# ChumpChief/FluidFramework

Measured on AMD Instinct MI355X. Metric: sequenced ops applied/sec (whole node) + achieved HBM GB/s, conflict-farm replay, higher is better.
Workload: dtype int32

## Files before the change

fluidframework_amd/csrc/mt_engine.h:

```cpp
#pragma once

#include "../../include/fmt.h"
#include "wave.h"
#include "adjust.h"
#include "huge_ckpt.h"

#include <cstddef>
#include <type_traits>

#if FMT_GPU
#define FMT_LDS __attribute__((address_space(3)))
#else
#define FMT_LDS
#endif

namespace fmt_mt {

constexpr int kMaxNodes = 8;
constexpr int kGranularity = 256;
constexpr int kObCap = 64;
constexpr int kKeysMax = FMT_MT_PROPS_KEYS_MAX;
constexpr int kKeyChunks = kKeysMax / 64;
static_assert(kKeysMax % 64 == 0, "prop-set slots come in whole waves");
constexpr int32_t kNotRemoved = 0x7fffffff;
constexpr int kCapacityFinal = -33;
constexpr int kCkptEscalate = -34;
constexpr int kCkptDescend = -36;
constexpr int kDescendLeaves4 = 128, kDescendChars4 = 1024;
constexpr int kDescendMinOps = 128;

struct SmallTier {
  static constexpr int kRows = 8;
  static constexpr int kCapChars = 6144;
  static constexpr int kMaxBlocks = 128;
  static constexpr int kHeapCap = 255;
  static constexpr int kPropCap = 32;
  static constexpr int kLenBits = 16, kBlkBits = 8;
  static constexpr bool kHbmChars = false;
  static constexpr bool kUnroll = true;
  static constexpr int kWords = 5;
  static constexpr int kMaxClient = 31;
  static constexpr bool kPropsWord = false;
  using BId = uint8_t;
  using VR = V8;
};

struct CompactTier : SmallTier {
  static constexpr int kRows = 4;
  static constexpr int kCapChars = 2048;
  using VR = V4;
};

struct MicroTier : SmallTier {
  static constexpr int kRows = 2;
  static constexpr int kCapChars = 1024;
  using VR = V2;
};

struct LargeTier {
  static constexpr int kRows = 32;
  static constexpr int kCapChars = 131071;
  static constexpr int kMaxBlocks = 1023;
  static constexpr int kHeapCap = 1023;
  static constexpr int kPropCap = 1024;
  static constexpr int kLenBits = 17, kBlkBits = 10;
  static constexpr bool kHbmChars = true;
  static constexpr bool kUnroll = false;
  static constexpr int kWords = 7;
  static constexpr int kMaxClient = 63;
  static constexpr bool kPropsWord = true;
  using BId = uint16_t;
  using VR = V32;
};

#define FMT_PRAGMA(x) _Pragma(#x)
#define FOR_ROWS(r, lo, hi)                                                                            \
  FMT_PRAGMA(unroll kRowUnroll)                                                                      \
  for (int r = kRowUnroll > 1 ? 0 : (lo); r < (kRowUnroll > 1 ? kRows : ((hi) < kRows ? (hi) : kRows)); r++) \
    if (r >= (lo) && r < (hi))
#define FOR_ROWS_DOWN(r, lo, hi)                                                                          \
  FMT_PRAGMA(unroll kRowUnroll)                                                                        \
  for (int r = kRowUnroll > 1 ? kRows - 1 : ((hi) < kRows ? (hi) : kRows) - 1; r >= (kRowUnroll > 1 ? 0 : (lo)); r--) \
    if (r >= (lo) && r < (hi))

template <class BId>
struct Blk {
  uint8_t count;
  BId parent;
  uint8_t leaf;
  int8_t needsScour;
  BId child[kMaxNodes];
};

struct HeapEnt {
  int32_t maxSeq;
  uint32_t leafId;
};

struct PropSet {
  uint32_t n;
  uint32_t kv[FMT_MT_PROPS_MAX];
};

struct ObEnt {
  uint32_t startId, endId;
  int32_t startOff, endOff;
  int32_t seq, client;
};

template <class C>
struct Scratch {
  uint16_t chars[C::kHbmChars ? 2 : C::kCapChars];
  Blk<typename C::BId> blk[C::kMaxBlocks];
  HeapEnt heap[C::kHeapCap + 1];
  PropSet props[C::kPropCap];
  uint16_t propCls[C::kPropCap];
  uint32_t kvWork[FMT_MT_PROPS_KEYS_MAX];
  typename C::BId freeList[C::kMaxBlocks];
  uint32_t tmp[64];
  ObEnt ob[kObCap];
  uint8_t obSeq[kObCap];
  uint8_t obStart[kObCap];
};

constexpr uint32_t kW4Marker = 1u << 23;
constexpr uint32_t kIdLimit = 1u << 23;
FMT_DEV uint32_t fId(uint32_t w4) { return w4 & 0x7FFFFFu; }
FMT_DEV bool fMarker(uint32_t w4) { return (w4 & kW4Marker) != 0; }
FMT_DEV int32_t fClient(uint32_t w4) { return static_cast<int32_t>(static_cast<int8_t>(w4 >> 24)); }
FMT_DEV uint32_t mkW4(uint32_t id, int32_t client) { return (id & 0x7FFFFFu) | (static_cast<uint32_t>(client & 0xFF) << 24); }

struct LeafRec {
  uint32_t w[8];
};

struct AdjustTables;

struct LocalTables {
  uint32_t* groups;
  const uint64_t* groupOffs;
  uint32_t* recs;
  const uint64_t* recOffs;
  uint32_t* pm;
  const uint64_t* pmOffs;
  fmt_mt_op* regen;
  const uint64_t* regenOffs;
  uint16_t* regenText;
  const uint64_t* regenTextOffs;
  uint32_t* regenCount;
  uint32_t* scratch;
  const uint64_t* scratchOffs;
};

struct DocInputs {
  const fmt_mt_op* ops;
  uint64_t begin, end;
  const uint16_t* text;
  uint32_t initOff, initLen;
  const uint32_t* propsOff;
  const uint32_t* propsKv;
  uint32_t nPropsOps;
  const fmt_mt_snapshot_seg* snapSegs;
  uint32_t nHeader, nBody;
  int32_t snapMinSeq, snapSeq;
  uint32_t loaded;
  const fmt_mt_snapshot_info* snapInfo;
  const fmt_mt_stamp* snapStamps;
  const fmt_mt_snapshot_info* infoAll;
  const fmt_mt_stamp* stampsAll;
  uint64_t nInfoAll;
  const fmt_mt_relpos* relpos;
  uint32_t nRelpos;
  uint32_t markerKey;
  const AdjustTables* adj;
  uint32_t doc;
  const LocalTables* loc = nullptr;
};

struct DocOutputs {
  fmt_mt_doc_result* header;
  fmt_mt_leaf* leaves;
  uint16_t* chars;
  fmt_mt_propset* props;
  fmt_mt_catchup_range* catchup;
  uint32_t catchupCap;
  fmt_mt_remove_order* rmOrder;
  uint32_t rmOrderCap;
  uint32_t* ckpt;
  bool ckptResume;
  uint32_t* bigCkpt;
  uint16_t* bigCkptChars;
  uint16_t* legacyProps;
  uint32_t* hugeCkpt = nullptr;
  bool descend = false;
};

#ifndef FMT_PROFILE
#define FMT_PROFILE 0
#endif
#ifndef FMT_SCALAR_OPS
#define FMT_SCALAR_OPS 0
#endif
enum ProfCat {
  kPfOpLoad, kPfScan, kPfSplit, kPfInsert, kPfRange, kPfLru, kPfZamboniOp, kPfWindow, kPfOutput,
  kPfInsChars, kPfInsShift, kPfZFind, kPfZChars, kPfZSerial, kPfZDelete, kPfZPack, kPfCount
};

template <bool Ob, class C = SmallTier, bool Rm = false, bool Adj = false, bool Loc = false>
class Doc {
 public:
  using VR = typename C::VR;
  using BId = typename C::BId;
  static constexpr int kRows = C::kRows;
  static constexpr int kRowUnroll = C::kUnroll ? C::kRows : 1;
  static constexpr int kCapLeaves = 64 * kRows;
  static constexpr int kCapChars = C::kCapChars;
  static constexpr int kMaxBlocks = C::kMaxBlocks;
  static constexpr int kHeapCap = C::kHeapCap;
  static constexpr int kPropCap = C::kPropCap;
  static constexpr uint32_t kLenMask = (1u << C::kLenBits) - 1u;
  static constexpr uint32_t kNoBlk = (1u << C::kBlkBits) - 1u;
  static constexpr bool kPW = C::kPropsWord;
  static constexpr int kCapFinal = C::kHbmChars ? FMT_E_CAPACITY : kCapacityFinal;
  static constexpr uint32_t kPropsUndef = kPW ? 0xFFFFu : (1u << (32 - C::kLenBits - C::kBlkBits)) - 1u;
  static_assert(kMaxBlocks <= static_cast<int>(kNoBlk) && kPropCap <= static_cast<int>(kPropsUndef), "W0 field widths");
  static_assert(kRows <= 32, "row bitmasks are 32-bit");
  FMT_DEV static uint32_t fLen(uint32_t w0) { return w0 & kLenMask; }
  FMT_DEV static uint32_t fBlk(uint32_t w0) { return (w0 >> C::kLenBits) & kNoBlk; }
  FMT_DEV static uint32_t fProps(uint32_t w0) { return kPW ? 0u : w0 >> (C::kLenBits + C::kBlkBits); }
  FMT_DEV static uint32_t mkW0(uint32_t len, uint32_t blk, uint32_t props) {
    return kPW ? len | (blk << C::kLenBits) : len | (blk << C::kLenBits) | (props << (C::kLenBits + C::kBlkBits));
  }

#if FMT_PROFILE && FMT_GPU
  uint64_t profT = 0;
  uint64_t prof[kPfCount] = {};
  FMT_DEV void stamp(int cat) {
    const uint64_t t = __builtin_amdgcn_s_memtime();
    prof[cat] += t - profT;
    profT = t;
  }
#else
  FMT_DEV void stamp(int) {}
#endif
  static constexpr int kWords = C::kWords + (Loc ? 1 : 0);
  static constexpr int kPropW = C::kWords - 1;
  static constexpr int kPendW = C::kWords;
  static constexpr int kMaxClient = C::kMaxClient;
  static constexpr int kTopClient = 253;
  Lane<VR> W[kWords];
  FMT_LDS Scratch<C>* s;
  uint16_t* gch = nullptr;
  int n = 0;
  int nChars = 0;
  int root = 0;
  int nFree = 0;
  int heapN = 0;
  int nProps = 0;
  int curSeq = 0;
  int minSeq = 0;
  int status = FMT_OK;
  int failSeq = 0;
  uint32_t nextId = 1;
  uint32_t opIdx = 0;
  int obSeqN = 0;
  int obStartN = 0;
  uint64_t obUsed = 0;
  uint32_t cuN = 0;
  DocInputs in;
  fmt_mt_catchup_range* cuOut = nullptr;
  uint32_t cuCap = 0;
  uint32_t rmN = 0;
  fmt_mt_remove_order* rmOut = nullptr;
  uint32_t rmCap = 0;
  int rmPendN = 0;
  uint32_t rmPendFrom0 = 0, rmPendTo0 = 0, rmPendFrom1 = 0, rmPendTo1 = 0;
  bool rmHitsSet = false;
  Lane<uint32_t> rmHits;

  static constexpr bool kRegTier = !C::kHbmChars && !Rm && !Loc;
  static constexpr bool kSavesCkpt = kRegTier && C::kRows < SmallTier::kRows;
  static constexpr bool kResumesCkpt = kRegTier && (C::kRows == SmallTier::kRows || (C::kRows > MicroTier::kRows && !Ob));
  static constexpr bool kDescends = kRegTier && !Ob && !Adj && C::kRows == SmallTier::kRows;
  static constexpr int kDescendLeaves = kDescendLeaves4;
  static constexpr int kDescendChars = kDescendChars4;
  static_assert(SmallTier::kMaxBlocks == CompactTier::kMaxBlocks && SmallTier::kPropCap == CompactTier::kPropCap &&
                    SmallTier::kMaxClient == CompactTier::kMaxClient && SmallTier::kHeapCap == CompactTier::kHeapCap &&
                    2 * kDescendLeaves4 <= 64 * CompactTier::kRows && 2 * kDescendChars4 <= CompactTier::kCapChars,
                "a document that steps down fits the compact tier with half of it to spare");
  bool descend = false;
  static constexpr int kCkptRows = CompactTier::kRows;
  static constexpr int kCkptHead = 16;
  static constexpr int kCkptCharWords = CompactTier::kCapChars / 2;
  static constexpr int kCkptRestWords =
      static_cast<int>((offsetof(Scratch<CompactTier>, tmp) - offsetof(Scratch<CompactTier>, blk) + 3) / 4);
  static_assert(offsetof(Scratch<CompactTier>, tmp) - offsetof(Scratch<CompactTier>, blk) ==
                    offsetof(Scratch<SmallTier>, tmp) - offsetof(Scratch<SmallTier>, blk),
                "checkpointed scratch fields");
  static constexpr int kCkptObWords =
      static_cast<int>((offsetof(Scratch<CompactTier>, obStart) + kObCap - offsetof(Scratch<CompactTier>, ob) + 3) / 4);
  static_assert(offsetof(Scratch<CompactTier>, obStart) - offsetof(Scratch<CompactTier>, ob) ==
                    offsetof(Scratch<SmallTier>, obStart) - offsetof(Scratch<SmallTier>, ob),
                "checkpointed obliterate fields");
  static constexpr int kCkptWords = kCkptHead + 5 * kCkptRows * 64 + kCkptCharWords + kCkptRestWords + kCkptObWords;
  uint32_t* ckpt = nullptr;
  uint64_t ckptNext = 0;

  static constexpr bool kSavesBig = !C::kHbmChars && C::kRows == SmallTier::kRows && !Rm && !Loc;
  static constexpr bool kResumesBig = C::kHbmChars && !Rm && !Loc;
  static constexpr int kCkptObOff = kCkptWords - kCkptObWords;
  static constexpr int kBigRows = SmallTier::kRows;
  static constexpr int kBigRestWords =
      static_cast<int>((offsetof(Scratch<SmallTier>, tmp) - offsetof(Scratch<SmallTier>, blk) + 3) / 4);
  static_assert(kCkptHead + 5 * kBigRows * 64 + kBigRestWords <= 64 * SmallTier::kRows * 8,
                "the small tier's checkpoint fits its leaves slab");
  uint32_t* bigCkpt = nullptr;
  uint16_t* bigCkptChars = nullptr;

  static constexpr bool kSavesHuge = C::kHbmChars && !Loc;
  uint32_t* hugeCkpt = nullptr;
  bool savingHuge = false;
  FMT_DEV void saveHuge(uint64_t next) {
    namespace K = fmt_ckpt;
    uint32_t* ck = hugeCkpt;
    FOR_LANES(l) {
      if (l == 0) {
        ck[K::kNextLo] = static_cast<uint32_t>(next);
        ck[K::kNextHi] = static_cast<uint32_t>(next >> 32);
        ck[K::kN] = static_cast<uint32_t>(n);
        ck[K::kNChars] = static_cast<uint32_t>(nChars);
        ck[K::kRoot] = static_cast<uint32_t>(root);
        ck[K::kNFree] = static_cast<uint32_t>(nFree);
        ck[K::kHeapN] = static_cast<uint32_t>(heapN);
        ck[K::kNProps] = static_cast<uint32_t>(nProps);
        ck[K::kCurSeq] = static_cast<uint32_t>(curSeq);
        ck[K::kMinSeq] = static_cast<uint32_t>(minSeq);
        ck[K::kNextId] = nextId;
        ck[K::kCuN] = cuN;
        ck[K::kObCounts] = Ob ? static_cast<uint32_t>(obSeqN) | (static_cast<uint32_t>(obStartN) << 16) : 0u;
        ck[K::kObUsedLo] = Ob ? static_cast<uint32_t>(obUsed) : 0u;
        ck[K::kObUsedHi] = Ob ? static_cast<uint32_t>(obUsed >> 32) : 0u;
        ck[K::kPmN] = Adj ? static_cast<uint32_t>(pmN) : 0u;
        ck[K::kRmN] = Rm ? rmN : 0u;
      }
    }
    static_assert(!kSavesHuge || (kCapLeaves == K::kLeaves && kMaxBlocks == K::kBlocks && kHeapCap + 1 == K::kHeap &&
                                  kObCap == K::kObSlots), "huge_ckpt.h layout");
    const int nr = rows();
    FOR_ROWS(r, 0, nr) {
      FOR_LANES(l) {
        const int j = r * 64 + l;
        if (j < n) {
          ck[K::kLeafW4 + j] = LANE(W[4])[r];
          ck[K::kLeafBlk + j] = fBlk(LANE(W[0])[r]);
        }
      }
    }
    FOR_LANES(l) {
      for (int b = l; b < kMaxBlocks; b += 64) {
        const Blk<BId> k = s->blk[b];
        uint32_t* o = ck + K::kBlk + K::kBlkWords * b;
        o[0] = static_cast<uint32_t>(k.count) | (static_cast<uint32_t>(k.leaf) << 8) |
               (static_cast<uint32_t>(static_cast<uint8_t>(k.needsScour)) << 16);
        o[1] = static_cast<uint32_t>(k.parent) == kNoBlk ? K::kNoParent : static_cast<uint32_t>(k.parent);
        for (int c = 0; c < kMaxNodes; c++) o[2 + c] = static_cast<uint32_t>(k.child[c]);
      }
      for (int k = l; k <= heapN; k += 64) {
        ck[K::kHeapOff + 2 * k] = static_cast<uint32_t>(s->heap[k].maxSeq);
        ck[K::kHeapOff + 2 * k + 1] = s->heap[k].leafId;
      }
      for (int k = l; k < nFree; k += 64) ck[K::kFree + k] = static_cast<uint32_t>(s->freeList[k]);
      if constexpr (Ob) {
        for (int k = l; k < kObCap; k += 64) {
          const ObEnt e = s->ob[k];
          uint32_t* o = ck + K::kOb + 6 * k;
          o[0] = e.startId;
          o[1] = e.endId;
          o[2] = static_cast<uint32_t>(e.startOff);
          o[3] = static_cast<uint32_t>(e.endOff);
          o[4] = static_cast<uint32_t>(e.seq);
          o[5] = static_cast<uint32_t>(e.client);
          ck[K::kObSeq + k] = s->obSeq[k];
          ck[K::kObStart + k] = s->obStart[k];
        }
      }
    }
    waveSync();
  }

  FMT_DEV void saveBig(uint64_t next) {
    uint32_t* ck = bigCkpt;
    FOR_LANES(l) {
      if (l == 0) {
        ck[0] = static_cast<uint32_t>(next);
        ck[1] = static_cast<uint32_t>(next >> 32);
        ck[2] = static_cast<uint32_t>(n);
        ck[3] = static_cast<uint32_t>(nChars);
        ck[4] = static_cast<uint32_t>(root);
        ck[5] = static_cast<uint32_t>(nFree);
        ck[6] = static_cast<uint32_t>(heapN);
        ck[7] = static_cast<uint32_t>(nProps);
        ck[8] = static_cast<uint32_t>(curSeq);
        ck[9] = static_cast<uint32_t>(minSeq);
        ck[10] = static_cast<uint32_t>(failSeq);
        ck[11] = nextId;
        ck[12] = cuN;
        if constexpr (Ob) {
          ck[13] = static_cast<uint32_t>(obSeqN) | (static_cast<uint32_t>(obStartN) << 16);
          ck[14] = static_cast<uint32_t>(obUsed);
          ck[15] = static_cast<uint32_t>(obUsed >> 32);
        }
      }
    }
    if constexpr (Ob) {
      const uint32_t* obw = reinterpret_cast<const FMT_LDS uint32_t*>(s->ob);
      FOR_LANES(l) {
        for (int t = l; t < kCkptObWords; t += 64) ckpt[kCkptObOff + t] = obw[t];
      }
    }
    FOR_LANES(l) {
#pragma unroll
      for (int f = 0; f < 5; f++) {
#pragma unroll
        for (int r = 0; r < kBigRows && r < kRows; r++) ck[kCkptHead + (f * kBigRows + r) * 64 + l] = LANE(W[f])[r];
      }
    }
    waveSync();
    const uint32_t* rest = reinterpret_cast<const uint32_t*>(reinterpret_cast<const unsigned char*>(s) + offsetof(Scratch<C>, blk));
    uint32_t* dst = ck + kCkptHead + 5 * kBigRows * 64;
    FOR_LANES(l) {
      for (int t = l; t < kBigRestWords; t += 64) dst[t] = rest[t];
      if constexpr (!C::kHbmChars)
        for (int t = l; t < nChars; t += 64) bigCkptChars[t] = s->chars[t];
    }
  }

  FMT_DEV uint64_t restoreBig() {
    const uint32_t* ck = bigCkpt;
    const uint64_t next = uni(ck[0]) | (static_cast<uint64_t>(uni(ck[1])) << 32);
    n = static_cast<int>(uni(ck[2]));
    nChars = static_cast<int>(uni(ck[3]));
    root = static_cast<int>(uni(ck[4]));
    const int smallFree = static_cast<int>(uni(ck[5]));
    heapN = static_cast<int>(uni(ck[6]));
    nProps = static_cast<int>(uni(ck[7]));
    curSeq = static_cast<int>(uni(ck[8]));
    minSeq = static_cast<int>(uni(ck[9]));
    failSeq = static_cast<int>(uni(ck[10]));
    nextId = uni(ck[11]);
    cuN = uni(ck[12]);
    if constexpr (Ob) {
      const uint32_t c13 = uni(ck[13]);
      obSeqN = static_cast<int>(c13 & 0xFFFFu);
      obStartN = static_cast<int>(c13 >> 16);
      obUsed = uni(ck[14]) | (static_cast<uint64_t>(uni(ck[15])) << 32);
      uint32_t* obw = reinterpret_cast<FMT_LDS uint32_t*>(s->ob);
      FOR_LANES(l) {
        for (int t = l; t < kCkptObWords; t += 64) obw[t] = ckpt[kCkptObOff + t];
      }
    }
    status = FMT_OK;
    constexpr uint32_t kSmallNoProps = 255u, kSmallNoBlk = 255u;
    FOR_ROWS(r, 0, kRows) {
      FOR_LANES(l) {
        uint32_t w[5] = {0u, 0u, 0u, 0u, 0u};
        if (r < kBigRows)
          for (int f = 0; f < 5; f++) w[f] = ck[kCkptHead + (f * kBigRows + r) * 64 + l];
        const bool live = r * 64 + l < n;
        const uint32_t sp = w[0] >> 24;
        LANE(W[0])[r] = live ? mkW0(w[0] & 0xFFFFu, (w[0] >> 16) & 0xFFu, 0u) : 0u;
        LANE(W[1])[r] = w[1];
        LANE(W[2])[r] = w[2];
        LANE(W[3])[r] = w[3];
        LANE(W[4])[r] = w[4];
        if constexpr (C::kWords > 5) {
          LANE(W[5])[r] = 0u;
          LANE(W[kPropW])[r] = live ? (sp == kSmallNoProps ? kPropsUndef : sp) : 0u;
        }
      }
    }
    const unsigned char* img = reinterpret_cast<const unsigned char*>(ck + kCkptHead + 5 * kBigRows * 64) -
                               offsetof(Scratch<SmallTier>, blk);
    const Scratch<SmallTier>* sm = reinterpret_cast<const Scratch<SmallTier>*>(img);
    const auto blkId = [&](uint32_t b) -> BId { return static_cast<BId>(b == kSmallNoBlk ? kNoBlk : b); };
    FOR_LANES(l) {
      for (int b = l; b < SmallTier::kMaxBlocks; b += 64) {
        const Blk<uint8_t> src = sm->blk[b];
        Blk<BId>& d = s->blk[b];
        d.count = src.count;
        d.parent = blkId(src.parent);
        d.leaf = src.leaf;
        d.needsScour = src.needsScour;
        for (int c = 0; c < kMaxNodes; c++) d.child[c] = blkId(src.child[c]);
      }
      for (int k = l; k <= heapN; k += 64) s->heap[k] = sm->heap[k];
      for (int k = l; k < nProps; k += 64) {
        s->props[k] = sm->props[k];
        s->propCls[k] = sm->propCls[k];
      }
      const int extra = kMaxBlocks - SmallTier::kMaxBlocks;
      for (int k = l; k < extra; k += 64) s->freeList[k] = static_cast<BId>(kMaxBlocks - 1 - k);
      for (int k = l; k < smallFree; k += 64) s->freeList[extra + k] = static_cast<BId>(sm->freeList[k]);
      if constexpr (C::kHbmChars)
        for (int t = l; t < nChars; t += 64) gch[t] = bigCkptChars[t];
// ... 2203 lines not shown
      if (op.type == FMT_MT_REMOVE) {
        if (isLocalSeq(readField(j, 2))) {
          writeField(j, 2, static_cast<uint32_t>(kNotRemoved));
          writeField(j, 3, 0u);
          if constexpr (C::kWords > 5) writeField(j, 5, 0u);
        }
      } else if (op.type == FMT_MT_INSERT) {
        if (readField(j, 2) != static_cast<uint32_t>(kNotRemoved)) {
          fail(FMT_E_DATA);
          return;
        }
        writeField(j, 1, static_cast<uint32_t>(-2));
        writeField(j, 2, static_cast<uint32_t>(-2));
        const uint32_t w4 = readField(j, 4);
        writeField(j, 4, mkW4(fId(w4), FMT_NON_COLLAB_CLIENT) | (w4 & kW4Marker));
        zamboni();
      } else {
        const bool removed = readField(j, 2) != static_cast<uint32_t>(kNotRemoved);
        locPmRollback(j, payload);
        if (!removed && status == FMT_OK) zamboni();
      }
    }
  }

  FMT_DEV void normalizeOnRebase() {
    uint32_t* S = in.loc->scratch + in.loc->scratchOffs[in.doc];
    const uint64_t cap = in.loc->scratchOffs[in.doc + 1] - in.loc->scratchOffs[in.doc];
    if (cap < 5ull * static_cast<uint64_t>(n) + 16ull) {
      fail(FMT_E_CAPACITY);
      return;
    }
    const int nr = rows();
    FOR_ROWS(r, 0, nr) {
      FOR_LANES(l) {
        const int j = r * 64 + l;
        if (j < n) {
          storeGlobal(S + j, LANE(W[1])[r]);
          storeGlobal(S + n + j, LANE(W[2])[r]);
        }
      }
    }
    waveSync();
    uint32_t* nxt = S + 2 * n;
    uint32_t* prv = S + 3 * n;
    const uint32_t kNil = 0xFFFFFFFFu;
    auto ins = [&](int j) { return uni(loadCoherent(S + j)); };
    auto rm = [&](int j) { return uni(loadCoherent(S + n + j)); };
    auto inRun = [&](int j) { return rm(j) != static_cast<uint32_t>(kNotRemoved) || isLocalSeq(ins(j)); };
    auto ackedRm = [&](int j) { return rm(j) != static_cast<uint32_t>(kNotRemoved) && !isLocalSeq(rm(j)); };
    auto put = [&](uint32_t* p, uint32_t v) {
      FOR_LANES(l) {
        if (l == 0) storeGlobal(p, v);
      }
      waveSync();
    };
    auto get = [&](const uint32_t* p) { return uni(loadCoherent(p)); };
    for (int a = 0; a < n && status == FMT_OK;) {
      if (!inRun(a)) {
        a++;
        continue;
      }
      int b = a;
      bool hasLocal = false, hasRemote = false;
      while (b < n && inRun(b)) {
        hasLocal = hasLocal || isLocalSeq(ins(b));
        hasRemote = hasRemote || ackedRm(b);
        b++;
      }
      const int m = b - a;
      if (hasLocal && hasRemote && m > 1) {
        for (int k = 0; k < m; k++) {
          put(nxt + k, k + 1 < m ? static_cast<uint32_t>(k + 1) : kNil);
          put(prv + k, k > 0 ? static_cast<uint32_t>(k - 1) : kNil);
        }
        uint32_t head = 0, tail = static_cast<uint32_t>(m - 1);
        auto unlink = [&](uint32_t x) {
          const uint32_t p = get(prv + x), q = get(nxt + x);
          if (p != kNil) put(nxt + p, q);
          else head = q;
          if (q != kNil) put(prv + q, p);
          else tail = p;
        };
        auto insertAfter = [&](uint32_t at, uint32_t x) {
          const uint32_t q = get(nxt + at);
          put(nxt + x, q);
          put(prv + x, at);
          put(nxt + at, x);
          if (q != kNil) put(prv + q, x);
          else tail = x;
        };
        uint32_t lastLocal = kNil;
        for (uint32_t x = tail; x != kNil; x = get(prv + x))
          if (!ackedRm(a + static_cast<int>(x))) {
            lastLocal = x;
            break;
          }
        if (lastLocal != kNil) {
          for (uint32_t slide = lastLocal;;) {
            const uint32_t nearer = get(prv + slide);
            const int sj = a + static_cast<int>(slide);
            if (ackedRm(sj)) {
              unlink(slide);
              insertAfter(lastLocal, slide);
            } else if (rm(sj) != static_cast<uint32_t>(kNotRemoved)) {
              uint32_t cur = slide;
              for (uint32_t scan = get(nxt + cur); scan != kNil; scan = get(nxt + scan)) {
                const int qj = a + static_cast<int>(scan);
                if (ackedRm(qj) || !isLocalSeq(ins(qj)) || ins(qj) <= rm(sj)) break;
                cur = scan;
              }
              if (cur != slide) {
                unlink(slide);
                insertAfter(cur, slide);
              }
            }
            if (nearer == kNil) break;
            slide = nearer;
          }
          uint32_t* perm = S + 4 * n;
          bool identity = true;
          int k = 0;
          for (uint32_t x = head; x != kNil; x = get(nxt + x), k++) {
            identity = identity && x == static_cast<uint32_t>(k);
            put(perm + k, x);
          }
          if (!identity) permuteRun(a, m, perm, S + 5 * n, cap - 5ull * static_cast<uint64_t>(n));
        }
      }
      a = b;
    }
  }

  FMT_DEV void permuteRun(int a, int m, const uint32_t* perm, uint32_t* area, uint64_t areaCap) {
    const int b = a + m;
    const uint32_t ca = charOffsetOf(a), cb = charOffsetOf(b);
    const uint64_t need = static_cast<uint64_t>(kWords) * m + static_cast<uint64_t>(m) + (cb - ca + 1) / 2 + 1;
    if (need > areaCap) {
      fail(FMT_E_CAPACITY);
      return;
    }
    uint32_t* R = area;
    uint32_t* co = area + static_cast<size_t>(kWords) * m;
    uint16_t* T = reinterpret_cast<uint16_t*>(co + m);
    const int r0 = a >> 6, r1 = ((b - 1) >> 6) + 1;
    FOR_ROWS(r, r0, r1) {
      FOR_LANES(l) {
        const int j = r * 64 + l;
        if (j >= a && j < b)
          for (int f = 0; f < kWords; f++) storeGlobal(R + static_cast<size_t>(j - a) * kWords + f, LANE(W[f])[r]);
      }
    }
    FOR_LANES(l) {
      for (uint32_t t = l; t < cb - ca; t += 64) storeGlobal(T + t, static_cast<uint16_t>(chRead(static_cast<int>(ca + t))));
    }
    waveSync();
    uint32_t off = 0;
    for (int k = 0; k < m; k++) {
      const uint32_t len = fLen(uni(loadCoherent(R + static_cast<size_t>(k) * kWords)));
      FOR_LANES(l) {
        if (l == 0) storeGlobal(co + k, off);
      }
      off += len;
    }
    waveSync();
    FOR_ROWS(r, r0, r1) {
      FOR_LANES(l) {
        const int j = r * 64 + l;
        if (j >= a && j < b) {
          const uint32_t src = loadCoherent(perm + (j - a));
          const uint32_t blk = fBlk(LANE(W[0])[r]);
          for (int f = 0; f < kWords; f++) {
            uint32_t v = loadCoherent(R + static_cast<size_t>(src) * kWords + f);
            if (f == 0) v = mkW0(fLen(v), blk, fProps(v));
            LANE(W[f])[r] = v;
          }
        }
      }
    }
    uint32_t dst = ca;
    for (int k = 0; k < m; k++) {
      const uint32_t src = uni(loadCoherent(perm + k));
      const uint32_t so = uni(loadCoherent(co + src));
      const uint32_t len = fLen(uni(loadCoherent(R + static_cast<size_t>(src) * kWords)));
      FOR_LANES(l) {
        for (uint32_t t = l; t < len; t += 64) chWrite(static_cast<int>(dst + t), loadCoherent(T + so + t));
      }
      dst += len;
    }
    waveSync();
  }

  FMT_DEV void regenerate() {
    if (gHead == gTail) return;
    if (!normSet || curSeq != normRef || locSeq != normLocal) {
      normalizeOnRebase();
      if (status != FMT_OK) return;
      normSet = true;
      normRef = curSeq;
      normLocal = locSeq;
    }
    if (gHead > 0) groupCompact();
    recCompact();
    recFrozen = true;
    const int g1 = gTail;
    fmt_mt_op* outOps = in.loc->regen + in.loc->regenOffs[in.doc];
    const uint32_t opCap = static_cast<uint32_t>(in.loc->regenOffs[in.doc + 1] - in.loc->regenOffs[in.doc]);
    uint16_t* outText = in.loc->regenText + in.loc->regenTextOffs[in.doc];
    const uint64_t textCap = in.loc->regenTextOffs[in.doc + 1] - in.loc->regenTextOffs[in.doc];
    for (int g = gHead; g < g1 && status == FMT_OK; g++) {
      const uint32_t ls = gWord(g, 0), tf = gWord(g, 1), payload = gWord(g, 2);
      const int32_t pos2 = static_cast<int32_t>(gWord(g, 3)), inflightRef = static_cast<int32_t>(gWord(g, 4));
      const int type = static_cast<int>(tf & 0xFFu);
      const int nr = rows();
      Lane<uint32_t> segs;
      FOR_LANES(l) { LANE(segs) = 0u; }
      for (int i = recFind(static_cast<uint32_t>(g), 0); i >= 0 && status == FMT_OK; i = recFind(static_cast<uint32_t>(g), i + 1)) {
        const int j = findLeafById(rWord(i, 0));
        if (j < 0) {
          fail(FMT_E_DATA);
          break;
        }
        rSet(i, 0, 0u);
        FOR_LANES(l) {
          if (l == (j & 63)) LANE(segs) |= 1u << (j >> 6);
        }
      }
      waveSync();
      if (status != FMT_OK) break;
      Lane<VR> vis, st;
      visLengths(static_cast<int>(FMT_MT_LOCAL_SEQ_BASE | ls), -5, vis, nr);
      scanRows(vis, st, nr);
      for (Lane<uint32_t> todo = segs; status == FMT_OK;) {
        const int j = firstSet(todo, nr);
        if (j < 0) break;
        FOR_LANES(l) {
          if (l == (j & 63)) LANE(todo) &= ~(1u << (j >> 6));
        }
        const uint32_t w1 = readField(j, 1), w2 = readField(j, 2), w4 = readField(j, 4);
        const uint32_t len = fLen(readField(j, 0));
        const int pos = static_cast<int>(readlane(selectRow(st, j >> 6), j & 63));
        const bool removed = w2 != static_cast<uint32_t>(kNotRemoved);
        bool emit = false;
        fmt_mt_op o;
        o.seq = static_cast<int32_t>(ls);
        o.ref_seq = curSeq;
        o.min_seq = 0;
        o.pos1 = pos;
        o.pos2 = pos + static_cast<int32_t>(len);
        o.payload = payload;
        o.len = 0;
        o.client = 0;
        o.type = static_cast<uint8_t>(type);
        o.flags = 0;
        if (type == FMT_MT_ANNOTATE) {
          emit = !(removed && !isLocalSeq(w2));
        } else if (type == FMT_MT_INSERT) {
          if (!isLocalSeq(w1)) {
            fail(FMT_E_DATA);
            break;
          }
          if (removed && !isLocalSeq(w2)) {
            fail(FMT_E_UNSUPPORTED);
            break;
          }
          if (regenTextN + len > textCap) {
            fail(FMT_E_CAPACITY);
            break;
          }
          const uint32_t c0 = charOffsetOf(j);
          FOR_LANES(l) {
            for (uint32_t t = l; t < len; t += 64) storeGlobal(outText + regenTextN + t, static_cast<uint16_t>(chRead(static_cast<int>(c0 + t))));
          }
          o.pos2 = pos2;
          o.payload = regenTextN;
          o.len = static_cast<uint16_t>(len & 0xFFFFu);
          o.flags = (len & FMT_MT_F_LEN_HI_MASK) | (fMarker(w4) ? FMT_MT_F_MARKER : 0u);
          regenTextN += len;
          emit = true;
        } else {
          emit = removed && isLocalSeq(w2);
        }
        if (emit) {
          if (regenN >= opCap) {
            fail(FMT_E_CAPACITY);
            break;
          }
          FOR_LANES(l) {
            if (l == 0) outOps[regenN] = o;
          }
          regenN++;
          const int ng = groupPush(ls, tf, payload, pos2, inflightRef);
          if (ng < 0) break;
          recAppend(fId(w4), static_cast<uint32_t>(ng));
        } else {
          pendAdd(j, -1);
        }
      }
    }
    waveSync();
    gHead = g1;
    recFrozen = false;
  }

  FMT_DEV int scourLeafBlock(int b) {
    const int cnt = uni(static_cast<int>(s->blk[b].count));
    if (cnt == 0) return 0;
    const int first = firstLeafOf(static_cast<uint32_t>(b));
    const int r0 = first >> 6, r1 = (first + cnt - 1) >> 6;
    Lane<uint32_t> pk0, pk1;
    Lane<uint32_t> pp0, pp1;
    FOR_LANES(l) {
      LANE(pk0) = 0u;
      LANE(pk1) = 0u;
      LANE(pp0) = 0u;
      LANE(pp1) = 0u;
    }
    uint32_t cs = charOffsetOf(first);
    uint32_t rowBase = cs;
    FOR_ROWS(r, r0, r1 + 1) {
      Lane<uint32_t> blen;
      FOR_LANES(l) {
        const int idx = r * 64 + l;
        LANE(blen) = idx >= first && idx < first + cnt ? fLen(LANE(W[0])[r]) : 0u;
      }
      uint32_t tot;
      const Lane<uint32_t> ex = waveExclusiveSum(blen, &tot);
      FOR_LANES(l) {
        const uint32_t w0 = LANE(W[0])[r];
        const int32_t ins = static_cast<int32_t>(LANE(W[1])[r]), rm = static_cast<int32_t>(LANE(W[2])[r]);
        const uint32_t bl = LANE(blen);
        const bool nl = bl > 0 && chRead(static_cast<int>(rowBase + LANE(ex) + bl - 1)) == 10u;
        const uint32_t pr = propsL(l, r);
        bool held = false;
        if constexpr (Loc) held = LANE(W[kPendW])[r] != 0u;
        const uint32_t p = fLen(w0) | ((kPW ? 0u : pr) << C::kLenBits) | (rm != kNotRemoved ? 1u << 24 : 0u) |
                           (rm <= minSeq ? 1u << 25 : 0u) | (ins <= minSeq ? 1u << 26 : 0u) | (nl ? 1u << 27 : 0u) |
                           (fMarker(LANE(W[4])[r]) ? 1u << 28 : 0u) | (held ? 1u << 29 : 0u);
        if (r == r0) LANE(pk0) = p;
        else LANE(pk1) = p;
        if constexpr (kPW) {
          if (r == r0) LANE(pp0) = pr;
          else LANE(pp1) = pr;
        }
      }
      rowBase += tot;
    }
    stamp(kPfZChars);
    uint32_t mergeMask = 0, dropMask = 0;
    int prev = -1;
    uint32_t prevLen = 0, prevProps = 0, prevBlk = 0;
    bool prevNl = false;
    int kept = 0;
    for (int k = 0; k < cnt; k++) {
      const int j = first + k;
      const uint32_t p = (j >> 6) == r0 ? readlane(pk0, j & 63) : readlane(pk1, j & 63);
      const uint32_t len = p & kLenMask;
      uint32_t props = (p >> C::kLenBits) & kPropsUndef;
      if constexpr (kPW) props = (j >> 6) == r0 ? readlane(pp0, j & 63) : readlane(pp1, j & 63);
      s->tmp[k] = cs;
      s->tmp[kMaxNodes + k] = len;
      if ((p >> 29) & 1u) {
        prev = -1;
        kept++;
      } else if (((p >> 24) & 1u) == 0) {
        if ((p >> 26) & 1u) {
          const bool lastNl = ((p >> 27) & 1u) != 0;
          const bool marker = ((p >> 28) & 1u) != 0;
          const bool canAppend = prev >= 0 && !prevNl && !marker &&
                                 (prevLen <= static_cast<uint32_t>(kGranularity) ||
                                  len <= static_cast<uint32_t>(kGranularity)) &&
                                 propsMatch(prevProps, props) && len > 0;
          if (canAppend) {
            mergeMask |= 1u << k;
            if constexpr (Ob) {
              if (obUsed != 0) obRefsMove(fId(readField(j, 4)), fId(readField(prev, 4)), 0, static_cast<int>(prevLen));
            }
            prevLen += len;
            prevNl = lastNl;
            writeField(prev, 0, mkW0(prevLen, prevBlk, prevProps));
          } else {
            prev = len > 0 && !marker ? j : -1;
            prevLen = len;
            prevProps = props;
            prevBlk = static_cast<uint32_t>(b);
            prevNl = lastNl;
            kept++;
          }
        } else {
          prev = -1;
          kept++;
        }
      } else {
        if ((p >> 25) & 1u) {
          dropMask |= 1u << k;
        } else {
          kept++;
        }
        prev = -1;
      }
      cs += len;
    }
    waveSync();
    stamp(kPfZSerial);
    if (dropMask != 0) {
      uint32_t c0 = 0, dropped = 0;
      for (int k = cnt - 1; k >= 0; k--)
        if ((dropMask >> k) & 1u) c0 = uni(s->tmp[k]);
      for (int k = 0; k < cnt; k++)
        if ((dropMask >> k) & 1u) dropped += uni(s->tmp[kMaxNodes + k]);
      const int newChars = nChars - static_cast<int>(dropped);
      for (int base = static_cast<int>(c0); base < newChars; base += 64) {
        Lane<uint32_t> v;
        FOR_LANES(l) {
          const int c = base + l;
          uint32_t shift = 0, before = 0;
          for (int k = 0; k < cnt; k++) {
            if ((dropMask >> k) & 1u) {
              const uint32_t ks = uni(s->tmp[k]), kl = uni(s->tmp[kMaxNodes + k]);
              if (static_cast<uint32_t>(c) >= ks - before) shift += kl;
              before += kl;
            }
          }
          LANE(v) = c < newChars ? chRead(c + static_cast<int>(shift)) : 0u;
        }
        waveSync();
        FOR_LANES(l) {
          if (base + l < newChars) chWrite(base + l, LANE(v));
        }
        waveSync();
      }
      nChars = newChars;
    }
    if constexpr (Adj || Loc) {
      for (uint32_t m = pmN > 0 ? (mergeMask | dropMask) : 0u; m != 0; m &= m - 1) pmDropLeaf(fId(readField(first + ctz32(m), 4)));
    }
    deleteLeaves(first, cnt, mergeMask | dropMask);
    stamp(kPfZDelete);
    return kept;
  }

  FMT_DEV void redistribute(int p, int total, bool leafLevel, int firstLeaf) {
    const int pc = uni(static_cast<int>(s->blk[p].count));
    for (int i = 0; i < pc; i++) freeBlk(uni(static_cast<int>(s->blk[p].child[i])));
    if (total > 0) {
      int nb = total / (kMaxNodes / 2);
      if (nb > kMaxNodes - 1) nb = kMaxNodes - 1;
      if (nb < 1) nb = 1;
      const int base = total / nb;
      int rem = total % nb;
      int consumed = 0;
      for (int q = 0; q < nb; q++) {
        int cnt = base;
        if (rem > 0) {
          cnt++;
          rem--;
        }
        const int id = allocBlk(leafLevel ? 1 : 0);
        if (id < 0) return;
        s->blk[id].count = static_cast<uint8_t>(cnt);
        s->blk[id].parent = static_cast<BId>(p);
        if (leafLevel) {
          tagLeaves(firstLeaf + consumed, cnt, static_cast<uint32_t>(id));
        } else {
          for (int k = 0; k < cnt; k++) {
            const int g = uni(static_cast<int>(s->tmp[consumed + k]));
            s->blk[id].child[k] = static_cast<BId>(g);
            s->blk[g].parent = static_cast<BId>(id);
          }
        }
        s->blk[p].child[q] = static_cast<BId>(id);
        waveSync();
        consumed += cnt;
      }
      s->blk[p].count = static_cast<uint8_t>(nb);
    } else {
      s->blk[p].count = 0;
      if (p == root) s->blk[p].leaf = 1;
    }
    waveSync();
    stamp(kPfZPack);
  }

  FMT_DEV void zamboni() {
    for (int i = 0; i < 2; i++) {
      if (heapN == 0) break;
      if constexpr (Adj) {
        if (pmN > 0) pmUpdateMsn(uni(s->heap[1].leafId), minSeq);
      }
      if (heapSeq(1) > minSeq) break;
      const HeapEnt ent = heapGet();
      const int j = findLeafById(ent.leafId);
      stamp(kPfZFind);
      if (j < 0) continue;
      const int b = static_cast<int>(fBlk(readField(j, 0)));
      if (uni(static_cast<int>(s->blk[b].needsScour)) == 0) continue;
      const int oldCount = uni(static_cast<int>(s->blk[b].count));
      int target = b, p = -1, ci = 0, total = 0, firstLeaf = -1;
      for (;;) {
        const int kept = scourLeafBlock(target);
        if (status != FMT_OK) return;
        if (p < 0) {
          s->blk[b].needsScour = 0;
          waveSync();
          if (kept >= oldCount) break;
          s->blk[b].count = static_cast<uint8_t>(kept);
          waveSync();
          const int parent = uni(static_cast<int>(s->blk[b].parent));
          if (kept >= kMaxNodes / 2 || parent == static_cast<int>(kNoBlk)) break;
          p = parent;
          ci = 0;
          target = uni(static_cast<int>(s->blk[p].child[0]));
          continue;
        }
        s->blk[target].count = static_cast<uint8_t>(kept);
        waveSync();
        if (kept > 0 && firstLeaf < 0) firstLeaf = firstLeafOf(static_cast<uint32_t>(target));
        total += kept;
        if (++ci < uni(static_cast<int>(s->blk[p].count))) {
          target = uni(static_cast<int>(s->blk[p].child[ci]));
          continue;
        }
        redistribute(p, total, true, firstLeaf);
        if (status != FMT_OK) return;
        for (;;) {
          const int pp = uni(static_cast<int>(s->blk[p].parent));
          if (uni(static_cast<int>(s->blk[p].count)) >= kMaxNodes / 2 || pp == static_cast<int>(kNoBlk)) break;
          p = pp;
          const int pc = uni(static_cast<int>(s->blk[p].count));
          int held = 0;
          for (int q = 0; q < pc; q++) {
            const int c = uni(static_cast<int>(s->blk[p].child[q]));
            const int cc = uni(static_cast<int>(s->blk[c].count));
            for (int k = 0; k < cc; k++) s->tmp[held++] = uni(static_cast<int>(s->blk[c].child[k]));
          }
          waveSync();
          redistribute(p, held, false, -1);
          if (status != FMT_OK) return;
        }
        break;
      }
    }
  }

  FMT_DEV void init() {
    n = 0;
    nChars = 0;
    heapN = 0;
    nProps = 0;
    curSeq = 0;
    minSeq = 0;
    status = FMT_OK;
    failSeq = 0;
    nextId = 1;
    obSeqN = 0;
    obStartN = 0;
    obUsed = 0;
    FOR_LANES(l) {
      VR z;
#pragma unroll
      for (int r = 0; r < kRows; r++) z[r] = 0u;
      LANE(W[0]) = z;
      LANE(W[1]) = z;
      LANE(W[2]) = z;
      LANE(W[3]) = z;
      if constexpr (C::kWords > 5) {
        LANE(W[5]) = z;
        LANE(W[kPropW]) = z;
      }
      LANE(W[4]) = z;
      if constexpr (Loc) LANE(W[kPendW]) = z;
    }
    FOR_LANES(l) {
      for (int i = l; i < kMaxBlocks; i += 64) s->freeList[i] = static_cast<BId>(kMaxBlocks - 1 - i);
    }
    waveSync();
    nFree = kMaxBlocks;
    root = allocBlk(1);
  }

  FMT_DEV void loadInitial() {
    const int len = static_cast<int>(in.initLen);
    if (len == 0) return;
    if (len > kCapChars || static_cast<uint32_t>(len) > kLenMask) {
      fail(FMT_E_CAPACITY);
      return;
    }
    const uint16_t* src = in.text + in.initOff;
    FOR_LANES(l) {
      for (int t = l; t < len; t += 64) chWrite(t, src[t]);
    }
    waveSync();
    nChars = len;
    const uint32_t w0 = mkW0(static_cast<uint32_t>(len), static_cast<uint32_t>(root), kPropsUndef);
    const uint32_t w4 = mkW4(nextId++, FMT_LOCAL_CLIENT);
    FOR_LANES(l) {
      if (l == 0) {
        LANE(W[0])[0] = w0;
        LANE(W[1])[0] = 0u;
        LANE(W[2])[0] = static_cast<uint32_t>(kNotRemoved);
        LANE(W[3])[0] = 0u;
        LANE(W[4])[0] = w4;
        if constexpr (kPW) LANE(W[kPropW])[0] = kPropsUndef;
      }
    }
    n = 1;
    s->blk[root].count = 1;
    waveSync();
  }

  FMT_DEV void appendLoadedChars(uint32_t off, uint32_t len) {
    FOR_LANES(l) {
      for (uint32_t t = l; t < len; t += 64) chWrite(nChars + static_cast<int>(t), in.text[off + t]);
    }
    waveSync();
    nChars += static_cast<int>(len);
  }

  FMT_DEV void loadProps(int first, int last) {
    FOR_ROWS(r, first >> 6, (last + 63) >> 6) {
      Lane<uint32_t> op;
      FOR_LANES(l) {
        const int j = r * 64 + l;
        LANE(op) = j >= first && j < last ? in.snapSegs[j].props : FMT_MT_NO_PROPS;
      }
      for (;;) {
        Lane<bool> p;
        FOR_LANES(l) { LANE(p) = LANE(op) != FMT_MT_NO_PROPS; }
        const uint64_t m = ballot(p);
        if (m == 0) break;
        const uint32_t id = readlane(op, ctz64(m));
        if (id >= in.nPropsOps) {
          fail(FMT_E_DATA);
          return;
        }
        const uint32_t pid = applyProps(kPropsUndef, id);
        if (status != FMT_OK) return;
        FOR_LANES(l) {
          if (LANE(op) == id) {
            setPropsL(l, r, pid);
            LANE(op) = FMT_MT_NO_PROPS;
          }
        }
      }
    }
  }

  FMT_DEV bool loadMergeInfo(int H, int N) {
    const int nr = (N + 63) >> 6;
    Lane<bool> bad, wide;
    FOR_LANES(l) {
      LANE(bad) = false;
      LANE(wide) = false;
    }
    FOR_ROWS(r, 0, nr) {
      FOR_LANES(l) {
        const int j = r * 64 + l;
        if (j < N) {
          const fmt_mt_snapshot_info inf = in.snapInfo[j];
          if (j >= H && (inf.ins_seq != 0 || inf.rm_count != 0)) LANE(bad) = true;
          int32_t rm = kNotRemoved;
          uint64_t mask = 0;
          for (uint32_t t = 0; t < inf.rm_count; t++) {
            const fmt_mt_stamp st = in.snapStamps[inf.rm_first + t];
            rm = st.seq < rm ? st.seq : rm;
            if (st.client < 0 || st.client > kMaxClient) LANE(wide) = true;
            else mask |= 1ull << st.client;
          }
          if (inf.ins_client > kMaxClient) LANE(wide) = true;
          LANE(W[1])[r] = static_cast<uint32_t>(inf.ins_seq);
          LANE(W[2])[r] = static_cast<uint32_t>(rm);
          LANE(W[3])[r] = static_cast<uint32_t>(mask);
          if constexpr (C::kWords > 5) LANE(W[5])[r] = static_cast<uint32_t>(mask >> 32);
          const uint32_t w4 = LANE(W[4])[r];
          LANE(W[4])[r] = mkW4(fId(w4), inf.ins_client) | (w4 & kW4Marker);
        }
      }
    }
    if (ballot(bad) != 0) {
      fail(FMT_E_UNSUPPORTED);
      return false;
    }
    if (ballot(wide) != 0) {
      fail(FMT_E_CAPACITY);
      return false;
    }
    return true;
  }

  FMT_DEV void loadSnapshot() {
    const int H = static_cast<int>(in.nHeader), N = static_cast<int>(in.nHeader + in.nBody);
    if (N > kCapLeaves) {
      fail(FMT_E_CAPACITY);
      return;
    }
    uint32_t chars = 0;
    for (int k = 0; k < N; k++) {
      const uint32_t len = uni(in.snapSegs[k].len) & ~FMT_MT_SEG_MARKER;
      if (len == 0) {
        fail(FMT_E_DATA);
        return;
      }
      chars += len;
    }
    if (chars > static_cast<uint32_t>(kCapChars)) {
      fail(FMT_E_CAPACITY);
      return;
    }
    uint32_t* stage = reinterpret_cast<FMT_LDS uint32_t*>(s->chars);
    if constexpr (!C::kHbmChars) {
      FOR_LANES(l) {
        for (int j = l; j < N; j += 64) stage[j] = in.snapSegs[j].len;
      }
      waveSync();
    }
#pragma unroll
    for (int r = 0; r < kRows; r++) {
      FOR_LANES(l) {
        const int j = r * 64 + l;
        const bool live = j < N;
        const uint32_t lenF = live ? (C::kHbmChars ? in.snapSegs[j].len : stage[j]) : 0u;
        const uint32_t len = lenF & ~FMT_MT_SEG_MARKER;
        LANE(W[0])[r] = live ? mkW0(len, static_cast<uint32_t>(j < H ? j / 7 : 0), kPropsUndef) : 0u;
        LANE(W[2])[r] = live ? static_cast<uint32_t>(kNotRemoved) : 0u;
        LANE(W[4])[r] = live ? mkW4(static_cast<uint32_t>(j + 1), FMT_NON_COLLAB_CLIENT) | ((lenF & FMT_MT_SEG_MARKER) != 0 ? kW4Marker : 0u) : 0u;
        if constexpr (kPW) LANE(W[kPropW])[r] = live ? kPropsUndef : 0u;
      }
    }
    waveSync();
    if (in.snapInfo != nullptr && !loadMergeInfo(H, N)) return;
    nextId = static_cast<uint32_t>(N + 1);
    if (H > 0) {
      int lo = 0, cnt = (H + 6) / 7;
      for (int b = 0; b < cnt; b++) {
        s->blk[b].count = static_cast<uint8_t>(H - 7 * b < 7 ? H - 7 * b : 7);
        s->blk[b].parent = static_cast<BId>(kNoBlk);
        s->blk[b].leaf = 1;
        s->blk[b].needsScour = -1;
      }
      waveSync();
      while (cnt > 1) {
        const int nb = (cnt + 6) / 7, nlo = lo + cnt;
        for (int q = 0; q < nb; q++) {
          const int id = nlo + q;
          const int c = cnt - 7 * q < 7 ? cnt - 7 * q : 7;
          s->blk[id].count = static_cast<uint8_t>(c);
          s->blk[id].parent = static_cast<BId>(kNoBlk);
          s->blk[id].leaf = 0;
          s->blk[id].needsScour = -1;
          for (int k = 0; k < c; k++) {
            s->blk[id].child[k] = static_cast<BId>(lo + 7 * q + k);
            s->blk[lo + 7 * q + k].parent = static_cast<BId>(id);
          }
        }
        waveSync();
        lo = nlo;
        cnt = nb;
      }
      root = lo;
      nFree = kMaxBlocks - (lo + 1);
    }
    n = H;
    minSeq = in.snapMinSeq;
    curSeq = in.snapSeq;
    for (int k = H; k < N; k++) {
      const int blk = n > 0 ? static_cast<int>(fBlk(readField(n - 1, 0))) : root;
      if (uni(static_cast<int>(s->blk[blk].count)) == 0) {
        s->blk[blk].leaf = 1;
        waveSync();
      }
      tagLeaves(k, 1, static_cast<uint32_t>(blk));
      n++;
      childAdded(blk);
      if (status != FMT_OK) return;
    }
    loadProps(0, N);
    for (int k = 0; k < N && status == FMT_OK; k++)
      appendLoadedChars(uni(in.snapSegs[k].text), uni(in.snapSegs[k].len) & ~FMT_MT_SEG_MARKER);
  }

#if FMT_SCALAR_OPS && FMT_GPU
  struct OpRec {
    uint32_t w[8];
  };
  FMT_DEV OpRec fetchOp(uint64_t i) const {
    OpRec r;
    typedef const __attribute__((address_space(4))) uint32_t* ConstPtr;
    if (i < in.end) {
      const uint64_t a = reinterpret_cast<uintptr_t>(in.ops + i);
      const uint64_t au = static_cast<uint32_t>(__builtin_amdgcn_readfirstlane(static_cast<int>(a))) |
                          (static_cast<uint64_t>(static_cast<uint32_t>(__builtin_amdgcn_readfirstlane(static_cast<int>(a >> 32)))) << 32);
      const ConstPtr p = (ConstPtr)(au);
#pragma unroll
      for (int k = 0; k < 8; k++) r.w[k] = p[k];
    } else {
#pragma unroll
      for (int k = 0; k < 8; k++) r.w[k] = 0u;
    }
    return r;
  }
  FMT_DEV static uint32_t recWord(const OpRec& r, int k) { return r.w[k]; }
#else
  using OpRec = Lane<uint32_t>;
// ... 348 lines not shown
```

Before: 534.3 million.

## Add ballot-based fast paths to skip scour work when nothing merges

scourLeafBlock now pre-scans the leaf rows with wave ballots to build drop and merge-eligibility masks. If no adjacent pair can merge and nothing is droppable, it returns early and skips the per-row char reads, prefix sums and the serial merge loop. If only drops exist, it derives the drop mask directly from the ballots and does a lighter serial length pass. The cost is an extra scan over all rows to locate the block's first leaf instead of calling firstLeafOf, which could be slower for large documents. A host-only counting hook is also added behind a compile flag.

New measurement: 542.1 million (median of 6 runs). 1.01x the previous value.

```diff
diff --git a/fluidframework_amd/csrc/mt_engine.h b/fluidframework_amd/csrc/mt_engine.h
--- a/fluidframework_amd/csrc/mt_engine.h
+++ b/fluidframework_amd/csrc/mt_engine.h
@@ -200,6 +200,14 @@
 #endif
 #ifndef FMT_SCALAR_OPS
 #define FMT_SCALAR_OPS 0
+#endif
+#if !FMT_GPU && defined(FMT_SCOUR_COUNT)
+extern "C" void fmtScourNote(int sibling, int pairs, int drops, uint32_t mergeMask, uint32_t dropMask);
+#define FMT_SCOUR_SLOW 1
+#define FMT_SCOUR_NOTE(sibling, pairs, drops, mergeMask, dropMask) fmtScourNote(sibling, pairs, drops, mergeMask, dropMask)
+#else
+#define FMT_SCOUR_SLOW 0
+#define FMT_SCOUR_NOTE(sibling, pairs, drops, mergeMask, dropMask) ((void)0)
 #endif
 enum ProfCat {
   kPfOpLoad, kPfScan, kPfSplit, kPfInsert, kPfRange, kPfLru, kPfZamboniOp, kPfWindow, kPfOutput,
@@ -3009,103 +3017,155 @@
     recFrozen = false;
   }
 
-  FMT_DEV int scourLeafBlock(int b) {
+  static constexpr bool kScourDropOnly = true;
+  FMT_DEV int scourLeafBlock(int b, [[maybe_unused]] bool sibling) {
     const int cnt = uni(static_cast<int>(s->blk[b].count));
     if (cnt == 0) return 0;
-    const int first = firstLeafOf(static_cast<uint32_t>(b));
-    const int r0 = first >> 6, r1 = (first + cnt - 1) >> 6;
-    Lane<uint32_t> pk0, pk1;
-    Lane<uint32_t> pp0, pp1;
-    FOR_LANES(l) {
-      LANE(pk0) = 0u;
-      LANE(pk1) = 0u;
-      LANE(pp0) = 0u;
-      LANE(pp1) = 0u;
-    }
+    int first = -1;
+    uint64_t dropB[2] = {0, 0}, elig[2] = {0, 0};
+    {
+      const int nr = rows();
+      int seen = 0;
+      FOR_ROWS(r, 0, nr) {
+        Lane<bool> inB;
+        FOR_LANES(l) { LANE(inB) = r * 64 + l < n && fBlk(LANE(W[0])[r]) == static_cast<uint32_t>(b); }
+        const uint64_t m = ballot(inB);
+        if (m != 0) {
+          const int k = first < 0 ? 0 : 1;
+          if (first < 0) first = r * 64 + ctz64(m);
+          Lane<bool> dp, ep;
+          FOR_LANES(l) {
+            const int32_t ins = static_cast<int32_t>(LANE(W[1])[r]), rm = static_cast<int32_t>(LANE(W[2])[r]);
+            bool held = false;
+            if constexpr (Loc) held = LANE(W[kPendW])[r] != 0u;
+            const int idx = r * 64 + l;
+            const bool in = idx >= first && idx < first + cnt;
+            LANE(dp) = in && rm != kNotRemoved && rm <= minSeq;
+            LANE(ep) = in && !held && rm == kNotRemoved && ins <= minSeq && !fMarker(LANE(W[4])[r]) &&
+                       fLen(LANE(W[0])[r]) > 0u;
+          }
+          dropB[k] = ballot(dp);
+          elig[k] = ballot(ep);
+          seen += __builtin_popcountll(m);
+          if (k == 1 || seen >= cnt) break;
+        }
+      }
+    }
+    const bool pairs = ((elig[0] & (elig[0] << 1)) | (elig[1] & (elig[1] << 1)) | ((elig[0] >> 63) & elig[1])) != 0;
+    const bool drops = (dropB[0] | dropB[1]) != 0;
+    if (!FMT_SCOUR_SLOW && !pairs && !drops) {
+      stamp(kPfZChars);
+      return cnt;
+    }
+    uint32_t mergeMask = 0, dropMask = 0;
+    int kept = 0;
     uint32_t cs = charOffsetOf(first);
-    uint32_t rowBase = cs;
-    FOR_ROWS(r, r0, r1 + 1) {
-      Lane<uint32_t> blen;
-      FOR_LANES(l) {
-        const int idx = r * 64 + l;
-        LANE(blen) = idx >= first && idx < first + cnt ? fLen(LANE(W[0])[r]) : 0u;
-      }
-      uint32_t tot;
-      const Lane<uint32_t> ex = waveExclusiveSum(blen, &tot);
-      FOR_LANES(l) {
-        const uint32_t w0 = LANE(W[0])[r];
-        const int32_t ins = static_cast<int32_t>(LANE(W[1])[r]), rm = static_cast<int32_t>(LANE(W[2])[r]);
-        const uint32_t bl = LANE(blen);
-        const bool nl = bl > 0 && chRead(static_cast<int>(rowBase + LANE(ex) + bl - 1)) == 10u;
-        const uint32_t pr = propsL(l, r);
-        bool held = false;
-        if constexpr (Loc) held = LANE(W[kPendW])[r] != 0u;
-        const uint32_t p = fLen(w0) | ((kPW ? 0u : pr) << C::kLenBits) | (rm != kNotRemoved ? 1u << 24 : 0u) |
-                           (rm <= minSeq ? 1u << 25 : 0u) | (ins <= minSeq ? 1u << 26 : 0u) | (nl ? 1u << 27 : 0u) |
-                           (fMarker(LANE(W[4])[r]) ? 1u << 28 : 0u) | (held ? 1u << 29 : 0u);
-        if (r == r0) LANE(pk0) = p;
-        else LANE(pk1) = p;
-        if constexpr (kPW) {
-          if (r == r0) LANE(pp0) = pr;
-          else LANE(pp1) = pr;
-        }
-      }
-      rowBase += tot;
-    }
-    stamp(kPfZChars);
-    uint32_t mergeMask = 0, dropMask = 0;
-    int prev = -1;
-    uint32_t prevLen = 0, prevProps = 0, prevBlk = 0;
-    bool prevNl = false;
-    int kept = 0;
-    for (int k = 0; k < cnt; k++) {
-      const int j = first + k;
-      const uint32_t p = (j >> 6) == r0 ? readlane(pk0, j & 63) : readlane(pk1, j & 63);
-      const uint32_t len = p & kLenMask;
-      uint32_t props = (p >> C::kLenBits) & kPropsUndef;
-      if constexpr (kPW) props = (j >> 6) == r0 ? readlane(pp0, j & 63) : readlane(pp1, j & 63);
-      s->tmp[k] = cs;
-      s->tmp[kMaxNodes + k] = len;
-      if ((p >> 29) & 1u) {
-        prev = -1;
-        kept++;
-      } else if (((p >> 24) & 1u) == 0) {
-        if ((p >> 26) & 1u) {
-          const bool lastNl = ((p >> 27) & 1u) != 0;
-          const bool marker = ((p >> 28) & 1u) != 0;
-          const bool canAppend = prev >= 0 && !prevNl && !marker &&
-                                 (prevLen <= static_cast<uint32_t>(kGranularity) ||
-                                  len <= static_cast<uint32_t>(kGranularity)) &&
-                                 propsMatch(prevProps, props) && len > 0;
-          if (canAppend) {
-            mergeMask |= 1u << k;
-            if constexpr (Ob) {
-              if (obUsed != 0) obRefsMove(fId(readField(j, 4)), fId(readField(prev, 4)), 0, static_cast<int>(prevLen));
-            }
-            prevLen += len;
-            prevNl = lastNl;
-            writeField(prev, 0, mkW0(prevLen, prevBlk, prevProps));
-          } else {
-            prev = len > 0 && !marker ? j : -1;
-            prevLen = len;
-            prevProps = props;
-            prevBlk = static_cast<uint32_t>(b);
-            prevNl = lastNl;
-            kept++;
-          }
-        } else {
+    if (!FMT_SCOUR_SLOW && kScourDropOnly && !pairs) {
+      const int f0 = first & 63;
+      dropMask = static_cast<uint32_t>((dropB[0] >> f0) | ((first >> 6) == ((first + cnt - 1) >> 6) ? 0ull : dropB[1] << (64 - f0))) &
+                 ((1u << cnt) - 1u);
+      kept = cnt - __builtin_popcount(dropMask);
+      for (int k = 0; k < cnt; k++) {
+        const uint32_t len = fLen(readField(first + k, 0));
+        if ((dropMask >> k) & 1u) {
+          s->tmp[k] = cs;
+          s->tmp[kMaxNodes + k] = len;
+        }
+        cs += len;
+      }
+      stamp(kPfZChars);
+    } else {
+      const int r0 = first >> 6, r1 = (first + cnt - 1) >> 6;
+      Lane<uint32_t> pk0, pk1;
+      Lane<uint32_t> pp0, pp1;
+      FOR_LANES(l) {
+        LANE(pk0) = 0u;
+        LANE(pk1) = 0u;
+        LANE(pp0) = 0u;
+        LANE(pp1) = 0u;
+      }
+      uint32_t rowBase = cs;
+      FOR_ROWS(r, r0, r1 + 1) {
+        Lane<uint32_t> blen;
+        FOR_LANES(l) {
+          const int idx = r * 64 + l;
+          LANE(blen) = idx >= first && idx < first + cnt ? fLen(LANE(W[0])[r]) : 0u;
+        }
+        uint32_t tot;
+        const Lane<uint32_t> ex = waveExclusiveSum(blen, &tot);
+        FOR_LANES(l) {
+          const uint32_t w0 = LANE(W[0])[r];
+          const int32_t ins = static_cast<int32_t>(LANE(W[1])[r]), rm = static_cast<int32_t>(LANE(W[2])[r]);
+          const uint32_t bl = LANE(blen);
+          const bool nl = bl > 0 && chRead(static_cast<int>(rowBase + LANE(ex) + bl - 1)) == 10u;
+          const uint32_t pr = propsL(l, r);
+          bool held = false;
+          if constexpr (Loc) held = LANE(W[kPendW])[r] != 0u;
+          const uint32_t p = fLen(w0) | ((kPW ? 0u : pr) << C::kLenBits) | (rm != kNotRemoved ? 1u << 24 : 0u) |
+                             (rm <= minSeq ? 1u << 25 : 0u) | (ins <= minSeq ? 1u << 26 : 0u) | (nl ? 1u << 27 : 0u) |
+                             (fMarker(LANE(W[4])[r]) ? 1u << 28 : 0u) | (held ? 1u << 29 : 0u);
+          if (r == r0) LANE(pk0) = p;
+          else LANE(pk1) = p;
+          if constexpr (kPW) {
+            if (r == r0) LANE(pp0) = pr;
+            else LANE(pp1) = pr;
+          }
+        }
+        rowBase += tot;
+      }
+      stamp(kPfZChars);
+      int prev = -1;
+      uint32_t prevLen = 0, prevProps = 0, prevBlk = 0;
+      bool prevNl = false;
+      for (int k = 0; k < cnt; k++) {
+        const int j = first + k;
+        const uint32_t p = (j >> 6) == r0 ? readlane(pk0, j & 63) : readlane(pk1, j & 63);
+        const uint32_t len = p & kLenMask;
+        uint32_t props = (p >> C::kLenBits) & kPropsUndef;
+        if constexpr (kPW) props = (j >> 6) == r0 ? readlane(pp0, j & 63) : readlane(pp1, j & 63);
+        s->tmp[k] = cs;
+        s->tmp[kMaxNodes + k] = len;
+        if ((p >> 29) & 1u) {
           prev = -1;
           kept++;
-        }
-      } else {
-        if ((p >> 25) & 1u) {
-          dropMask |= 1u << k;
+        } else if (((p >> 24) & 1u) == 0) {
+          if ((p >> 26) & 1u) {
+            const bool lastNl = ((p >> 27) & 1u) != 0;
+            const bool marker = ((p >> 28) & 1u) != 0;
+            const bool canAppend = prev >= 0 && !prevNl && !marker &&
+                                   (prevLen <= static_cast<uint32_t>(kGranularity) ||
+                                    len <= static_cast<uint32_t>(kGranularity)) &&
+                                   propsMatch(prevProps, props) && len > 0;
+            if (canAppend) {
+              mergeMask |= 1u << k;
+              if constexpr (Ob) {
+                if (obUsed != 0) obRefsMove(fId(readField(j, 4)), fId(readField(prev, 4)), 0, static_cast<int>(prevLen));
+              }
+              prevLen += len;
+              prevNl = lastNl;
+              writeField(prev, 0, mkW0(prevLen, prevBlk, prevProps));
+            } else {
+              prev = len > 0 && !marker ? j : -1;
+              prevLen = len;
+              prevProps = props;
+              prevBlk = static_cast<uint32_t>(b);
+              prevNl = lastNl;
+              kept++;
+            }
+          } else {
+            prev = -1;
+            kept++;
+          }
         } else {
-          kept++;
-        }
-        prev = -1;
-      }
-      cs += len;
+          if ((p >> 25) & 1u) {
+            dropMask |= 1u << k;
+          } else {
+            kept++;
+          }
+          prev = -1;
+        }
+        cs += len;
+      }
     }
     waveSync();
     stamp(kPfZSerial);
@@ -3141,6 +3201,7 @@
     if constexpr (Adj || Loc) {
       for (uint32_t m = pmN > 0 ? (mergeMask | dropMask) : 0u; m != 0; m &= m - 1) pmDropLeaf(fId(readField(first + ctz32(m), 4)));
     }
+    FMT_SCOUR_NOTE(sibling, pairs, drops, mergeMask, dropMask);
     deleteLeaves(first, cnt, mergeMask | dropMask);
     stamp(kPfZDelete);
     return kept;
@@ -3204,7 +3265,7 @@
       const int oldCount = uni(static_cast<int>(s->blk[b].count));
       int target = b, p = -1, ci = 0, total = 0, firstLeaf = -1;
       for (;;) {
-        const int kept = scourLeafBlock(target);
+        const int kept = scourLeafBlock(target, p >= 0);
         if (status != FMT_OK) return;
         if (p < 0) {
           s->blk[b].needsScour = 0;
```
